# iucario/WorkoutDetector

Hardware: AMD Instinct MI355X
Metric: clips/sec (8x3x224x224 TSM-R50) (higher is better)
Workload: dtype f32

## Files before the change

workoutdetector_amd/csrc/tsm_conv_rules.h:

```cpp
#pragma once
#include <stdint.h>
#include <string.h>

#if defined(__HIPCC__)
#define TSM_HOST_DEVICE __host__ __device__
#else
#define TSM_HOST_DEVICE
#endif

namespace tsm {

struct ConvParams {
  const float *x;
  const float *w;
  const float *bias;
  const float *res;
  float *y;
  int N, Hi, Wi, C, logC4;
  int Ho, Wo, Cout;
  int stride, pad;
  int Kp;
  int M;
  int relu;
  int T;
  int fold;
  int ntm, ntn;
  int tile;
  int prec;
  const float *x2;
  int C2, Hi2, Wi2, stride2;
  int K1;
  int kseg_len;
  int ksplit;
  int tail_from;
  float *ypart;
  int reverse;
  int pos_major;
};

enum ConvPrec { kPrecF32 = 0, kPrecBf16x3 = 1, kPrecBf16 = 2 };
constexpr int kPrecBlockShift = 4;
constexpr int kPrecPosMajor = 8;

enum ConvTile {
  kTileAuto = 0, kTile128x128 = 1, kTile128x64 = 2, kTile64x64 = 3, kTile32x32 = 4,
  kTile128x128w8 = 5,
  kTile256x256 = 6,
  kTileWs = 7,
  kTile256x256p = 8,
  kNumTiles = 9
};

struct Fused23Params {
  const float *x;
  const float *w2;
  const float *bias2;
  const float *w3f;
  const float *bias3;
  const float *res;
  float *y;
  int N, H, W;
  int M;
  int kseg_len;
  int reverse;
};

struct BneckParams {
  const void *x;
  const void *w1;
  const float *bias1;
  const void *w2;
  const float *bias2;
  const void *w3;
  const float *bias3;
  void *y;
  int cin;
  int N, H, W;
  int T, fold;
  int reverse;
};

struct FrontParams {
  const void *x;
  const void *w1;
  const float *bias1;
  const void *w2;
  const float *bias2;
  void *y;
  int N, H, W;
  int T, fold;
  int reverse;
};

struct Conv31Params {
  const void *t2;
  const void *w3;
  const float *bias3;
  const void *res;
  void *y;
  const void *w1;
  const float *bias1;
  void *t1;
  int n_clips, T, HW;
  int K3, C, N1;
  int fold;
  int reverse;
  int log_px;
};

constexpr int kBK = 32;

inline void conv_tile_dims(int tile, int *bm, int *bn) {
  *bm = (tile == kTile256x256 || tile == kTile256x256p || tile == kTileWs) ? 256 : tile == kTile32x32 ? 32 : (tile == kTile64x64 ? 64 : 128);
  *bn = (tile == kTile256x256 || tile == kTile256x256p) ? 256 : tile == kTile32x32 ? 32 : ((tile == kTile128x128 || tile == kTile128x128w8) ? 128 : 64);
}

inline int conv_tile_from_name(const char *name) {
  if (!name) return kTileAuto;
  static const struct { const char *n; int t; } names[] = {{"128x128", kTile128x128}, {"128x64", kTile128x64},
      {"64x64", kTile64x64}, {"32x32", kTile32x32}, {"128x128w8", kTile128x128w8}, {"256x256", kTile256x256}, {"ws", kTileWs}, {"256x256p", kTile256x256p}};
  for (const auto &e : names)
    if (strcmp(name, e.n) == 0) return e.t;
  return kTileAuto;
}

inline int conv_num_segments(const ConvParams &p) {
  if (p.kseg_len <= 0) return 1;
  const int nk = p.Kp / kBK;
  return (int)(((long)nk + p.kseg_len - 1) / p.kseg_len);
}

inline void conv_tile_shape(const ConvParams &p, int *bm, int *bn) {
  const int bn128 = p.Cout % 128 == 0 ? 128 : 64;
  const bool few = (((long)p.M + 127) / 128) * (p.Cout / bn128) < 256;
  *bm = few ? 64 : 128;
  *bn = few ? 64 : bn128;
}

constexpr int kWsRounds = 11;
constexpr int kWsPatchMax = kWsRounds * 32;
constexpr int kW8Rounds = 6;
constexpr int kW8PatchMax = kW8Rounds * 32;
constexpr int kS2PatchMax = 289;

inline bool ws_tile_geometry(int H, int W, int *tr_out, int *tc_out, int max_px = 256, int max_patch = kWsPatchMax) {
  long best_tiles = -1;
  int best_tr = 0, best_tc = 0, best_patch = 0;
  for (int tc = 4; tc <= 128; ++tc) {
    int tr = max_px / tc;
    if (tr > H) tr = H;
    if (tr < 1) continue;
    const int patch = (tr + 2) * (tc + 2);
    if (patch > max_patch) continue;
// ... 165 lines not shown
inline bool conv1x1_ws_valid(const ConvParams &p) {
  return p.prec == kPrecBf16 && (p.C == 64 || p.C == 256) && p.Cout == 64 && p.Kp == p.C && p.stride == 1 && p.pad == 0 &&
         p.Hi == p.Ho && p.Wi == p.Wo && !p.res && !p.x2 && p.kseg_len == 0 && (double)p.M * 128.0 < 2.0e9 &&
         (p.T == 0 || (p.N % p.T == 0 && p.fold % 8 == 0 && 2 * (int64_t)p.fold <= p.C)) &&
         (double)(128 + 2.0 * p.Hi * p.Wi) * p.C * 2.0 < 2.0e9;
}
inline bool conv1x1_wsn_valid(const ConvParams &p, int n_cu) {
  if (p.prec != kPrecBf16 || p.stride != 1 || p.pad != 0 || p.Hi != p.Ho || p.Wi != p.Wo || p.res || p.kseg_len != 0) return false;
  if ((double)(128 + 2.0 * p.Hi * p.Wi) * p.C * 2.0 >= 2.0e9) return false;
  if (p.x2) {
    const bool l1 = p.C == 64 && p.C2 == 64 && p.K1 == 64 && p.Kp == 128 && p.Cout == 256;
    const bool l2 = p.C == 128 && p.C2 == 256 && p.K1 == 128 && p.Kp == 384 && p.Cout == 512 && n_cu >= 16;
    return p.T == 0 && (l1 || l2) && (double)(128.0 / ((double)p.Hi * p.Wi) + 2.0) * p.Hi2 * p.Wi2 * p.C2 * 2.0 < 2.0e9;
  }
  if (p.Kp != p.C) return false;
  if (p.T > 0 && (p.N % p.T != 0 || p.fold % 8 != 0 || 2 * (int64_t)p.fold > p.C)) return false;
  return (p.C == 256 && p.Cout == 128) || (p.C == 512 && p.Cout == 128) || (p.C == 512 && p.Cout == 256);
}

inline bool conv_tile_valid(const ConvParams &p, int tile, int n_cu) {
  if (p.T > 0 && (p.res || p.x2 || (p.pad == 0 && p.stride != 1)) &&
      (tile == kTile256x256 || tile == kTileWs || (tile == kTile256x256p && (p.pad != 0 || !(p.res || p.x2)))))
    return false;
  switch (tile) {
    case kTile128x128: return p.Cout % 128 == 0;
    case kTile128x64:
    case kTile64x64: return p.Cout % 64 == 0;
    case kTile32x32: return p.Cout % 32 == 0 && p.prec == kPrecF32;
    case kTile128x128w8: return p.Cout % 128 == 0;
    case kTile256x256:
    case kTile256x256p:
      return p.prec == kPrecBf16 && p.Cout % 256 == 0 && p.C % 64 == 0 && !(p.res && p.x2) && (p.pad != 1 || (!p.res && p.T == 0)) &&
             (!p.x2 || (p.K1 % 64 == 0 && p.C2 % 64 == 0)) && (tile == kTile256x256 || (p.Cout <= 2048 && p.Kp >= 128));
    case kTileWs: {
      int tr, tc;
      return conv3x3_ws_valid(p, &tr, &tc) || conv3x3_ws128s2_valid(p, &tr, &tc) || conv3x3_ws128_valid(p, &tr, &tc, nullptr) ||
             conv1x1_ws_valid(p) || conv1x1_wsn_valid(p, n_cu);
    }
    default: return false;
  }
}

enum ConvFamily { kFamInvalid = 0, kFamIgemm, kFamIgemmSeg, kFamBf16_256, kFamBf16_256p, kFamWs3x3, kFamWs128, kFamWs128s2, kFamWs1x1, kFamWsn };

struct ConvRoute {
  int family = kFamInvalid, ks = 0;
  int bm = 0, bn = 0, wgm = 0, wgn = 0;
  bool shift = false, res = false, dual = false, block_shift = false;
  bool pos_major = false;
  int ntm = 0, ntn = 0;
  long tiles = 0;
  unsigned grid = 0;
  int tr = 0, tc = 0, swz = 0;
};

inline bool conv_args_refused(const ConvParams &p, int ks) {
  const int kc = p.prec == kPrecBf16 ? 64 : kBK;
  if (p.Cout % 64 != 0 || p.Kp % kc != 0 || p.M <= 0) return true;
  if (p.logC4 < 0 || p.logC4 > 28 || (1 << p.logC4) * 4 != p.C) return true;
  if (ks != 7 && p.C % kc != 0) return true;
  if (p.T > 0 && ((ks != 1 && ks != 3) || (ks == 3 && p.kseg_len > 0) || p.N % p.T != 0 || p.fold % 4 != 0 ||
                  (p.res && 2 * (int64_t)p.fold > p.Cout) || (p.x2 && 2 * (int64_t)p.fold > p.C2)))
    return true;
  if (p.x2 && (ks != 1 || p.res || p.K1 % kc != 0 || p.C2 % kc != 0 || (int64_t)p.K1 + p.C2 != p.Kp || p.K1 != p.C))
    return true;
  if (p.x2 && (128.0 / ((double)p.Ho * p.Wo) + 4.0) * (double)p.Hi2 * p.Wi2 * p.C2 * 4.0 > 2.0e9) return true;
// ... 47 lines not shown
  else conv_tile_dims(p.tile, &r.bm, &r.bn);
  if (p.tile == kTile256x256 || p.tile == kTile256x256p) {
    const bool persistent = p.tile == kTile256x256p;
    if (!(persistent ? conv_bf16_256p_valid(p, ks) : conv_bf16_256_valid(p, ks))) return refused;
    r.family = persistent ? kFamBf16_256p : kFamBf16_256;
    r.wgm = 2; r.wgn = 4;
    r.shift = ks == 1 && p.T > 0;
    r.ntm = (int)(((long)p.M + 255) / 256); r.ntn = p.Cout / 256;
    r.tiles = (long)r.ntm * r.ntn;
    const int slots = n_cu & ~7;
    r.grid = (unsigned)(!persistent || r.tiles < slots || slots < 8 ? r.tiles : slots);
    return r.tiles > 0x7fffffffL ? refused : r;
  }
  if (p.tile == kTileWs) {
    if (ks == 3) {
      r.family = conv3x3_ws128s2_valid(p, &r.tr, &r.tc) ? kFamWs128s2 : conv3x3_ws128_valid(p, &r.tr, &r.tc, &r.swz) ? kFamWs128 :
                 conv3x3_ws_valid(p, &r.tr, &r.tc) ? kFamWs3x3 : kFamInvalid;
      if (r.family == kFamInvalid) return refused;
      if (r.family == kFamWs128s2) r.swz = ws128s2_swap(r.tr, r.tc);
      r.tiles = ws_frame_tiles(p.N, p.Ho, p.Wo, r.tr, r.tc);
    } else {
      r.family = ks != 1 || r.res ? kFamInvalid : conv1x1_ws_valid(p) ? kFamWs1x1 : conv1x1_wsn_valid(p, n_cu) ? kFamWsn : kFamInvalid;
      if (r.family == kFamInvalid) return refused;
      const int px = r.family == kFamWs1x1 || p.Kp <= 256 ? 128 : 64;
      r.tiles = ((long)p.M + px - 1) / px;
    }
    r.grid = persistent_grid(r.tiles, n_cu);
    if (r.family == kFamWsn && p.x2 && p.Kp == 384) {
      const int pairs = n_cu >> 4 << 3;
      r.grid = 2u * (unsigned)(r.tiles < pairs ? (r.tiles + 7) / 8 * 8 : pairs);
    }
    return r;
  }
  if (p.kseg_len > 0 && r.bm != 32) r.bm = r.bn = 64;
  if (r.bm == 32 && p.prec != kPrecF32) return refused;
  r.wgm = r.bm == 32 ? 1 : r.bm == 128 && r.bn == 128 && p.tile == kTile128x128w8 ? 4 : 2;
  r.wgn = r.bm == 32 ? 1 : 2;
  r.ntm = (int)(((long)p.M + r.bm - 1) / r.bm); r.ntn = p.Cout / r.bn;
  r.tiles = (long)r.ntm * r.ntn;
  long grid = r.tiles;
  if (p.kseg_len > 0) {
    if (r.res || ks == 7 || (r.shift && ks == 3)) return refused;
    if (p.ksplit == 2 && (p.tail_from <= 0 || p.tail_from >= r.tiles || p.tail_from % r.ntn != 0)) return refused;
    r.family = kFamIgemmSeg;
    r.pos_major = p.pos_major != 0 && r.bm == 64 && pos_major_valid(p, ks);
    grid = p.ksplit == 2 ? p.tail_from + (r.tiles - p.tail_from) * conv_num_segments(p) : r.tiles * (p.ksplit ? conv_num_segments(p) : 1);
  } else {
    r.family = kFamIgemm;
  }
  r.block_shift = p.T > 0 && (r.dual || r.res);
  r.grid = (unsigned)grid;
  return grid > 0x7fffffffL ? refused : r;
}

inline bool conv23_ws_valid(int n, int h, int w, int *tr_out = nullptr, int *tc_out = nullptr) {
  int tr, tc;
  return n > 0 && h > 0 && w > 0 && (double)h * w * 512.0 < 2.0e9 && (double)n * h * w < 2.0e9 &&
         ws_tile_geometry(h, w, tr_out ? tr_out : &tr, tc_out ? tc_out : &tc);
}
inline bool bneck_ws_valid(int cin, int n, int h, int w, int T, int fold) {
  return (cin == 256 || cin == 64) && n > 0 && h > 0 && w >= 1 && w <= 64 && (double)h * w * 512.0 * 3.0 < 2.0e9 &&
         (T == 0 || (T > 0 && n % T == 0 && fold == cin / 8));
}
inline bool front_s2_valid(int n, int h, int w, int T, int fold) {
  return n > 0 && h >= 2 && (h & 1) == 0 && w >= 2 && w <= 64 && (double)h * w * 512.0 * 3.0 < 2.0e9 &&
         (T == 0 || (T > 0 && n % T == 0 && fold == 32));
// ... 16 lines not shown
```

workoutdetector_amd/csrc/tsm_engine.hip:

```cpp
#include <hip/hip_runtime.h>

#include <sys/stat.h>

#include <algorithm>
#include <cerrno>
#include <cmath>
#include <cstdio>
#include <cstdlib>
#include <cstring>
#include <map>
#include <string>
#include <vector>

#include "../../include/tsm_hip.h"
#include "tsm_host_util.h"
#include "tsm_kernels.h"

#ifndef TSM_BUILD_ID
#define TSM_BUILD_ID __DATE__ "/" __TIME__
#endif

namespace {

using namespace tsm_host;
// ... 142 lines not shown
  hipStream_t stream = nullptr;
  bool finalized = false;
  int prec = tsm::kPrecF32;
  float *d_tap = nullptr;
  std::map<std::string, HostTensor> tensors;
  std::vector<ConvLayer> convs;
  std::vector<Block> blocks;
  float *d_fcw = nullptr, *d_fcb = nullptr;
  float *d_in = nullptr;
  float *d_in4 = nullptr;
  float *buf[5] = {nullptr, nullptr, nullptr, nullptr, nullptr};
  float *d_pooled = nullptr, *d_logits = nullptr;
  float *d_partial = nullptr;
  size_t partial_elems = 0;
  size_t buf_elems = 0;
  int h1 = 0, w1 = 0, hp = 0, wp = 0;
  hipEvent_t ev0 = nullptr, ev1 = nullptr;
  bool have_time = false;
  std::vector<void *> allocs;
  bool poison = false;
  std::vector<GuardBuf> guards;
  std::map<int, std::vector<int>> tile_cache;
  bool autotune = true;
  bool stem_pool = true;
  bool stem_direct = true;
  bool stem_planar = true;
  std::string tune_path, tune_sig;
  int force_tile = 0, force_code = -1;
  int fuse23 = -1;
  int fuse_block = -1;
  int fuse31 = -1;
  int fuse_front = -1;
  bool pos_major = true;
  int walk = -1;
  int n_cu = 256;
  int timing_left = 0;
  bool timing_only3x3 = false;
  std::vector<std::vector<hipEvent_t>> timing;
  std::vector<hipEvent_t> event_pool;
  std::vector<hipEvent_t> *cur_timing = nullptr;
};

namespace {

int fail(tsm_engine *e, int code, const std::string &msg) {
  if (e) e->err = msg; else g_create_error = msg;
  return code;
}

#define TSM_HIP(e, call)                                                                        \
  do {                                                                                          \
    hipError_t _st = (call);                                                                    \
    if (_st != hipSuccess)                                                                      \
      return fail((e), TSM_ERR_HIP, std::string(#call) + ": " + hipGetErrorString(_st));        \
  } while (0)

int add_conv(tsm_engine *e, const std::string &wkey, const std::string &bnp, int cin, int cout, int k, int stride, bool segmented) {
  ConvLayer c;
  static_cast<LayerGeom &>(c) = layer_geometry(cin, k, stride, e->prec);
  if (!segmented) c.kseg = 0;
  c.wkey = wkey; c.bnp = bnp; c.cin = cin; c.cout = cout; c.k = k; c.stride = stride;
  e->convs.push_back(c);
  return (int)e->convs.size() - 1;
}

void build_convnext_topology(tsm_engine *e) {
// ... 580 lines not shown

hipError_t Forward::launch_code(tsm::ConvParams p, int ks, int code) {
  return launch_conv_code(p, ks, code, e->d_partial, e->partial_elems, e->n_cu, s);
}

int Forward::conv(int idx, tsm::ConvParams p, int ks, bool is3x3) {
  p.reverse = next_dir();
  if (!tuning) {
    int code = tiles ? (*tiles)[idx] : 0;
    if (e->force_tile) code = e->force_tile;
    if (e->force_code >= 0) code = e->force_code;
    TSM_LAUNCH_K(e, s, is3x3, launch_code(p, ks, checked_code(p, code, e->n_cu)));
    return TSM_OK;
  }
  std::vector<int> cands;
  if (p.kseg_len > 0) {
    const size_t need = (size_t)tsm::conv_num_segments(p) * p.M * p.Cout;
    const long tiles64 = (long)((p.M + 63) / 64) * (p.Cout / 64);
    for (int t : {(int)tsm::kTile64x64, (int)tsm::kTile32x32}) {
      cands.push_back(t);
      if (need <= e->partial_elems && tiles64 < 4L * e->n_cu) cands.push_back(t | kCodeSplitK);
    }
    int tail_from = 0;
    const bool tail = tail_split_from(p, e->n_cu, e->partial_elems, &tail_from);
    if (tail) cands.push_back((int)tsm::kTile64x64 | kCodeTailK);
    tsm::ConvParams q = p;
    q.tile = tsm::kTile64x64;
    if (e->pos_major && tsm::pos_major_valid(q, ks)) {
      cands.push_back((int)tsm::kTile64x64 | kCodePosMajor);
      if (tail) cands.push_back((int)tsm::kTile64x64 | kCodePosMajor | kCodeTailK);
    }
  } else {
    for (int t = 1; t < tsm::kNumTiles; ++t)
      if (tsm::conv_tile_valid(p, t, e->n_cu)) cands.push_back(t);
  }
  float best_ms = 0.f;
  int best = 0;
  for (int t : cands) {
    float ms = 0.f;
    const int rc = time_best_of(e, s, [&] { return launch_code(p, ks, t); }, &ms);
    if (rc) return rc;
    if (best == 0 || ms < best_ms) {
      best = t;
      best_ms = ms;
    }
  }
  (*tiles)[idx] = best;
  return TSM_OK;
}

int Forward::run_basic(size_t k, int nn, float *x, float *y, int hh, int ww) {
  const Block &blk = e->blocks[k];
  const std::string &name = blk.name;
  const ConvLayer &c1 = e->convs[blk.conv1], &c2 = e->convs[blk.conv2];
  const int T = blk.T, shiftT = e->cfg.is_shift ? T : 0;
  const int ho = conv_out_size(hh, 3, blk.stride), wo = conv_out_size(ww, 3, blk.stride);
  const float *identity = x;
  if (blk.down >= 0) {
    tsm::ConvParams pd = make_params(e->convs[blk.down], x, nullptr, idb, nn, hh, ww, false, block_shift(e) ? shiftT : 0,
                                     e->cfg.shift_div, prec);
    int rcd = conv(blk.down, pd, 1, false);
    if (rcd) return rcd;
    identity = idb;
  }
  tsm::ConvParams p1 = make_params(c1, x, nullptr, t1, nn, hh, ww, true, shiftT, e->cfg.shift_div, prec);
  int rc1 = conv(blk.conv1, p1, 3, true);
  if (rc1) return rc1;
// ... 854 lines not shown
  if (!cfg || !out) return fail(nullptr, TSM_ERR_INVALID_ARG, "cfg/out is NULL");
  *out = nullptr;
  if (cfg->struct_size != (int32_t)sizeof(tsm_config))
    return fail(nullptr, TSM_ERR_INVALID_ARG, "tsm_config.struct_size mismatch (ABI)");
  if (cfg->num_class <= 0 || cfg->num_segments <= 0 || cfg->max_clips <= 0)
    return fail(nullptr, TSM_ERR_INVALID_ARG, "num_class, num_segments, max_clips must be positive");
  if (cfg->height < 32 || cfg->width < 32)
    return fail(nullptr, TSM_ERR_INVALID_ARG, "height/width must be >= 32");
  {
    const int64_t rows = (int64_t)cfg->max_clips * cfg->num_segments * ((cfg->height + 1) / 2) * ((cfg->width + 1) / 2);
    if (rows >= (int64_t)1 << 31)
      return fail(nullptr, TSM_ERR_CAPACITY, "max_clips * num_segments * (H/2) * (W/2) must stay below 2^31");
  }
  if (const char *why = shift_div_refusal(cfg->shift_div, tsm::kPrecF32)) return fail(nullptr, TSM_ERR_UNSUPPORTED, why);
  if (prec_of_dtype(cfg->dtype) < 0)
    return fail(nullptr, TSM_ERR_UNSUPPORTED, "dtype must be TSM_DTYPE_F32, TSM_DTYPE_BF16X3 or TSM_DTYPE_BF16");
  if (const char *why = shift_div_refusal(cfg->shift_div, prec_of_dtype(cfg->dtype))) return fail(nullptr, TSM_ERR_UNSUPPORTED, why);
  int ndev = 0;
  hipError_t st = hipGetDeviceCount(&ndev);
  if (st != hipSuccess || ndev <= 0)
    return fail(nullptr, TSM_ERR_HIP, std::string("no HIP device: ") + hipGetErrorString(st));
  if (cfg->device_id < 0 || cfg->device_id >= ndev) return fail(nullptr, TSM_ERR_INVALID_ARG, "bad device_id");
  tsm_engine *e = new tsm_engine();
  e->cfg = *cfg;
  e->prec = prec_of_dtype(cfg->dtype);
  const auto on = [](const char *s) { return atoi(s) != 0; };
  env_read("TSM_AUTOTUNE", &e->autotune, on);
  env_read("TSM_STEM_DIRECT", &e->stem_direct, on);
  env_read("TSM_STEM_POOL", &e->stem_pool, on);
  env_read("TSM_STEM_PLANAR", &e->stem_planar, on);
  env_read("TSM_CONV_TILE", &e->force_tile, tsm::conv_tile_from_name);
  env_read("TSM_CONV_CODE", &e->force_code, atoi);
  env_read("TSM_POS_MAJOR", &e->pos_major, on);
  env_read("TSM_FUSE_CONV23", &e->fuse23, on);
  env_read("TSM_FUSE_BLOCK", &e->fuse_block, on);
  env_read("TSM_FUSE_C3C1", &e->fuse31, on);
  env_read("TSM_FUSE_FRONT", &e->fuse_front, on);
  env_read("TSM_WALK", &e->walk, on);
  env_read("TSM_POISON", &e->poison, on);
  const char *tc = getenv("TSM_TUNE_CACHE");
  if (!tc) e->tune_path = default_tune_cache_path();
  else if (*tc && strcmp(tc, "0") != 0 && strcmp(tc, "off") != 0) e->tune_path = tc;
  build_topology(e);
  st = hipSetDevice(cfg->device_id);
  if (st == hipSuccess) st = hipStreamCreateWithFlags(&e->stream, hipStreamNonBlocking);
  if (st == hipSuccess) st = hipDeviceGetAttribute(&e->n_cu, hipDeviceAttributeMultiprocessorCount, cfg->device_id);
  if (st == hipSuccess) st = hipEventCreate(&e->ev0);
  if (st == hipSuccess) st = hipEventCreate(&e->ev1);
  if (st != hipSuccess) {
    g_create_error = std::string("engine init: ") + hipGetErrorString(st);
    delete e;
    return TSM_ERR_HIP;
  }
  if (!e->tune_path.empty()) {
    hipDeviceProp_t prop;
    e->tune_sig = "abi" + std::to_string(TSM_ABI_VERSION) + " build " TSM_BUILD_ID " " +
                  (hipGetDeviceProperties(&prop, cfg->device_id) == hipSuccess ? std::string(prop.gcnArchName) : "?") +
                  " cu" + std::to_string(e->n_cu) +
                  " T" + std::to_string(cfg->num_segments) + " " + std::to_string(cfg->height) + "x" +
                  std::to_string(cfg->width) + " dtype" + std::to_string(cfg->dtype) + " shift" +
                  std::to_string(cfg->is_shift ? cfg->shift_div : 0) + " fuse" + std::to_string(e->fuse23) + "/" + std::to_string(e->fuse_block) + "/" + std::to_string(e->fuse31) + "/" + std::to_string(e->fuse_front) +
                  " stem" + std::to_string(e->stem_direct ? 1 : 0) +
                  std::to_string(e->stem_pool ? 1 : 0) + std::to_string(e->stem_planar ? 1 : 0);
    e->tune_sig_base = e->tune_sig.size();
  }
  *out = e;
// ... 764 lines not shown
```

workoutdetector_amd/csrc/tsm_igemm.hip:

```cpp
#include "tsm_device.h"

namespace tsm {

template <int BM, int BN, int WGM, int WGN, int KS, bool SHIFT, bool RES, int PREC, bool DUAL = false, bool SEG = false>
__global__ void __launch_bounds__(64 * WGM * WGN, (SEG && BM == 64) ? ((PREC & kPrecBlockShift) ? 4 : 5) : 1)
conv_igemm(const ConvParams p) {
  constexpr bool BSHIFT = (PREC & kPrecBlockShift) != 0;
  constexpr bool POSM = (PREC & kPrecPosMajor) != 0;
  constexpr int PMODE = PREC & ~(kPrecBlockShift | kPrecPosMajor);
  static_assert(!POSM || (SEG && KS == 3 && BM == 64 && BN == 64 && !SHIFT && !RES && !DUAL && !BSHIFT && PMODE == kPrecF32),
                "position-major rows: the segmented fp32 3x3 on 64x64 tiles only (pos_major_valid)");
  static_assert(!BSHIFT || (!SHIFT && !RES), "block placement: a shifted identity (DUAL = false) or a shifted second source");
  constexpr bool RESID = RES || (BSHIFT && !DUAL);
  static_assert(!SEG || (PMODE == kPrecF32 && !RES && WGM * WGN <= 4 && BM == BN && BM <= 64),
                "segmented K accumulation: fp32, 64x64 / 32x32 tiles, no residual (ConvParams::kseg_len)");
  static_assert(WGM * WGN == 4 || WGM * WGN == 1 || WGM * WGN == 8,
                "4 waves per workgroup, 1 (32x32 small-M tiles) or 8 (128x128 with 4 waves per SIMD at 2 workgroups/CU)");
  constexpr int NT = 64 * WGM * WGN;
  constexpr int LRP = NT / 8;
  static_assert(!DUAL || (KS == 1 && !SHIFT && !RES), "K-concatenated second source: plain 1x1 convs only");
  constexpr bool X3 = PMODE == kPrecBf16x3;
  constexpr bool BF = PMODE == kPrecBf16;
  constexpr int EB = BF ? 2 : 4;
  constexpr int KC = 128 / EB;
  static_assert(!SHIFT || KS == 1 || (KS == 3 && !SEG), "the temporal shift is fused into 1x1 and unsegmented 3x3 convs only");
  constexpr int WTM = BM / WGM, WTN = BN / WGN;
  constexpr int TM = WTM / 32, TN = WTN / 32;
  constexpr int APASS = BM / LRP, BPASS = BN / LRP;
  constexpr bool RK = PMODE == kPrecF32 && ((BM == 64 && BN == 64) || (BM == 32 && BN == 32));
  constexpr int NBUF = RK ? 1 : 2;
  constexpr int CLD = BN + 4;
  static_assert(TM >= 1 && TN >= 1, "wave tile must hold at least one 32x32 MFMA tile");
  constexpr int SMEM_FLOATS = NBUF * (BM + BN) * kLds > BM * CLD ? NBUF * (BM + BN) * kLds : BM * CLD;

  __shared__ __attribute__((aligned(16))) float smem[SMEM_FLOATS];

  const int tid = threadIdx.x;
  const int lane = tid & 63;
  const int wave = tid >> 6;
  const int wm = wave / WGN, wn = wave % WGN;
  const int half = lane >> 5, l31 = lane & 31;

  const int bid = blockIdx.x;
  const bool tail_mode = SEG && p.ksplit == 2;
  const bool in_tail = tail_mode && bid >= p.tail_from;
  const int nwg = tail_mode ? p.tail_from : (int)gridDim.x;
  const int q = nwg >> 3, r = nwg & 7, xcd = bid & 7;
  int tile = (xcd < r ? xcd * (q + 1) : r * (q + 1) + (xcd - r) * q) + (bid >> 3);
  if (p.reverse) tile = nwg - 1 - tile;
  int seg = 0;
  if (SEG && p.ksplit == 1) {
    seg = tile / (p.ntm * p.ntn);
    tile -= seg * (p.ntm * p.ntn);
  }
  if (in_tail) {
    const int u = bid - p.tail_from, n_tail = p.ntm * p.ntn - p.tail_from;
    seg = u / n_tail;
    tile = p.tail_from + (u - seg * n_tail);
  }
  const bool split_wg = SEG && (p.ksplit == 1 || in_tail);
  const int tm = tile / p.ntn, tn = tile - tm * p.ntn;
  const int m0 = tm * BM, n0 = tn * BN;

  const int HoWo = p.Ho * p.Wo;
// ... 253 lines not shown
  u32x4 af16[4][TM], bf16f[4][TN];
  auto frag_load_bf = [&](int buf, int qg) {
    const float *As = smem + buf * (BM + BN) * kLds + (wm * WTM + l31) * kLds + qg * 8 + half * 4;
    const float *Bs = smem + buf * (BM + BN) * kLds + BM * kLds + (wn * WTN + l31) * kLds + qg * 8 + half * 4;
#pragma unroll
    for (int i = 0; i < TM; ++i) af16[qg][i] = *reinterpret_cast<const u32x4 *>(As + i * 32 * kLds);
#pragma unroll
    for (int j = 0; j < TN; ++j) bf16f[qg][j] = *reinterpret_cast<const u32x4 *>(Bs + j * 32 * kLds);
  };
  constexpr int NMFMA_BF = TM * TN;
  auto mfma_bf = [&](int qg, int item0, int nitems, auto &&inject) {
    int cnt = 0;
#pragma unroll
    for (int i = 0; i < TM; ++i)
#pragma unroll
      for (int j = 0; j < TN; ++j) {
        acc[i][j] = __builtin_amdgcn_mfma_f32_32x32x16_bf16(__builtin_bit_cast(bf16x8, af16[qg][i]),
                                                            __builtin_bit_cast(bf16x8, bf16f[qg][j]), acc[i][j], 0, 0, 0);
        ++cnt;
        const int done = (cnt * nitems) / NMFMA_BF, before = ((cnt - 1) * nitems) / NMFMA_BF;
#pragma unroll
        for (int it = before; it < done; ++it) {
          inject(item0 + it);
          __builtin_amdgcn_sched_barrier(0);
        }
      }
  };

  constexpr int EW = (X3 || BF) ? 8 : 4;
  constexpr int TPR = BN / EW;
  constexpr int RPP = NT / TPR;
  constexpr int EPASS = BM / RPP;
  const int ecol = (tid % TPR) * EW, erow = tid / TPR;
  f32x4 rres[(RESID && !X3 && !BF) ? EPASS : 1];
  u32x4 rres_h[(RESID && (X3 || BF)) ? EPASS : 1], rres_l[(RESID && X3) ? EPASS : 1];
  if (RESID && (X3 || BF) && !BSHIFT) {
    const size_t r_bytes = ((size_t)p.M - m0) * p.Cout * EB;
    const __amdgpu_buffer_rsrc_t rsrcR = buffer_window(reinterpret_cast<const char *>(p.res) + (size_t)m0 * p.Cout * EB, r_bytes);
#pragma unroll
    for (int k = 0; k < EPASS; ++k) {
      const unsigned o = (unsigned)(((erow + k * RPP) * p.Cout + n0 + ecol) * EB);
      rres_h[k] = __builtin_amdgcn_raw_buffer_load_b128(rsrcR, (int)o, 0, 0);
      if (X3) rres_l[k] = __builtin_amdgcn_raw_buffer_load_b128(rsrcR, (int)(o + 16), 0, 0);
    }
  }
  if (RESID && !X3 && !BF && !BSHIFT) {
    const size_t r_bytes = ((size_t)p.M - m0) * p.Cout * 4;
    const __amdgpu_buffer_rsrc_t rsrcR = buffer_window(p.res + (size_t)m0 * p.Cout, r_bytes);
#pragma unroll
    for (int k = 0; k < EPASS; ++k)
      rres[k] = buf_load4(rsrcR, (unsigned)(((erow + k * RPP) * p.Cout + n0 + ecol) * 4), 0);
  }
  if constexpr (RESID && BSHIFT) {
    const int rbase = m0 >= HoWo ? m0 - HoWo : 0;
    const int c = n0 + ecol;
    const int sel = c < p.fold ? 1 : c < 2 * p.fold ? -1 : 0;
    const unsigned step = (unsigned)(HoWo * p.Cout * EB);
    const size_t r_bytes = ((size_t)p.M - rbase) * p.Cout * EB;
    const __amdgpu_buffer_rsrc_t rsrcR = buffer_window(reinterpret_cast<const char *>(p.res) + (size_t)rbase * p.Cout * EB, r_bytes);
#pragma unroll
    for (int k = 0; k < EPASS; ++k) {
      const int rr = erow + k * RPP;
      const int t = ((m0 + rr) / HoWo) % p.T;
      unsigned o = (unsigned)(((m0 - rbase + rr) * p.Cout + c) * EB);
      if (sel > 0) o = t < p.T - 1 ? o + step : kInvalid;
      if (sel < 0) o = t > 0 ? o - step : kInvalid;
      if constexpr (X3 || BF) {
        rres_h[k] = __builtin_amdgcn_raw_buffer_load_b128(rsrcR, (int)o, 0, 0);
        if (X3) rres_l[k] = __builtin_amdgcn_raw_buffer_load_b128(rsrcR, (int)(o + 16), 0, 0);
      } else {
        rres[k] = buf_load4(rsrcR, o, 0);
      }
    }
  }

  int kt0 = 0, nk = p.Kp / KC;
  if (split_wg) {
    kt0 = seg * p.kseg_len;
    nk = kt0 + p.kseg_len < nk ? kt0 + p.kseg_len : nk;
// ... 28 lines not shown
#pragma unroll
    for (int it = 0; it < NITEMS; ++it) gload_item(k0, pm_first, it);
#pragma unroll
    for (int it = 0; it < NITEMS; ++it) lstore_item(0, it);
    const KStep k1 = kstep(pm_second, nk);
#pragma unroll
    for (int it = 0; it < NITEMS; ++it) gload_item(k1, pm_second, it);
  }
  __syncthreads();
  if constexpr (BF) {
    frag_load_bf(0, 0);
    frag_load_bf(0, 1);
    for (int kt = kt0; kt < nk; ++kt) {
      const int cur = (kt - kt0) & 1;
      const KStep k2 = kstep(kt + 2, nk);
      frag_load_bf(cur, 2);
      frag_load_bf(cur, 3);
      auto inject = [&](int it) {
        if (it < NITEMS) lstore_item(cur ^ 1, it);
        else gload_item(k2, kt + 2, it - NITEMS);
      };
      mfma_bf(0, 0, NITEMS, inject);
      mfma_bf(1, NITEMS, NITEMS, inject);
      __syncthreads();
      __builtin_amdgcn_sched_barrier(0);
      mfma_bf(2, 0, 0, [](int) {});
      frag_load_bf(cur ^ 1, 0);
      __builtin_amdgcn_sched_barrier(0);
      mfma_bf(3, 0, 0, [](int) {});
      __builtin_amdgcn_sched_barrier(0);
      frag_load_bf(cur ^ 1, 1);
      __builtin_amdgcn_sched_barrier(0);
    }
  } else if constexpr (RK) {
    f32x4 ra_[4], rb_[4];
    const bool trim = KS == 7 && p.Kp == 224 && nk == 7;
    const int nk_full = trim ? nk - 1 : nk;
    if constexpr (POSM) {
      int kt = pm_first, kt1 = pm_second;
      while (kt < nk) {
        const int bound = (kt / seg_len + 1) * seg_len, kend = bound < nk ? bound : nk;
        while (kt < kend) {
          const int kt2 = next_live_kstep(kt1 + 1, pm_live, pm_spt, nk);
          const KStep k2 = kstep(kt2, nk);
          {
            const float *As = smem + (wm * WTM + l31) * kLds + half * 4;
            const float *Bs = smem + BM * kLds + (wn * WTN + l31) * kLds + half * 4;
#pragma unroll
            for (int kk = 0; kk < 4; ++kk) {
              ra_[kk] = *reinterpret_cast<const f32x4 *>(As + kk * 8);
              rb_[kk] = *reinterpret_cast<const f32x4 *>(Bs + kk * 8);
            }
          }
          __syncthreads();
          int cnt = 0;
#pragma unroll
          for (int kk = 0; kk < 4; ++kk)
#pragma unroll
            for (int s4 = 0; s4 < 4; ++s4) {
              acc[0][0] = __builtin_amdgcn_mfma_f32_32x32x2f32(ra_[kk][s4], rb_[kk][s4], acc[0][0], 0, 0, 0);
              ++cnt;
              const int done = cnt < 12 ? (cnt * 2 * NITEMS) / 12 : 2 * NITEMS;
              const int before = cnt - 1 < 12 ? ((cnt - 1) * 2 * NITEMS) / 12 : 2 * NITEMS;
#pragma unroll
              for (int it = before; it < done; ++it) {
                if (it < NITEMS) lstore_item(0, it);
// ... 203 lines not shown
        if (r.block_shift) TSM_KLAUNCH_WALK(p.reverse, (conv_igemm<BM, BN, WGM, WGN, 1, false, false, kPrecF32 | kPrecBlockShift, true, true>), grid, block, 0, s, p);
        else TSM_KLAUNCH_WALK(p.reverse, (conv_igemm<BM, BN, WGM, WGN, 1, false, false, kPrecF32, true, true>), grid, block, 0, s, p);
        return hipGetLastError();
      }
    }
    if constexpr (BM == 64 && WGM == 2 && KS == 3 && !SHIFT) {
      if (r.pos_major) {
        TSM_KLAUNCH_WALK(p.reverse, (conv_igemm<64, 64, 2, 2, 3, false, false, kPrecF32 | kPrecPosMajor, false, true>), grid, block, 0, s, p);
        return hipGetLastError();
      }
    }
    TSM_KLAUNCH_WALK(p.reverse, (conv_igemm<BM, BN, WGM, WGN, KS, SHIFT, false, kPrecF32, false, true>), grid, block, 0, s, p);
    return hipGetLastError();
  }
}

template <int BM, int BN, int WGM, int WGN, int KS, bool SHIFT, bool RES>
static hipError_t launch_conv_t(const ConvParams &p, const ConvRoute &r, hipStream_t s) {
  if (r.family == kFamIgemmSeg) {
    if constexpr (!RES && KS != 7 && !(SHIFT && KS == 3)) return launch_conv_seg<BM, BN, WGM, WGN, KS, SHIFT>(p, r, s);
    else return hipErrorInvalidValue;
  }
  const dim3 grid(r.grid), block(64 * WGM * WGN);
  if constexpr (KS == 1 && !SHIFT && !RES) {
    if (r.dual && r.block_shift) TSM_LAUNCH_IGEMM_AND_RETURN(TSM_ARM_DUAL_SHIFT);
    if (r.dual) TSM_LAUNCH_IGEMM_AND_RETURN(TSM_ARM_DUAL);
  }
  if constexpr (RES && !SHIFT && KS != 7) {
    if (r.block_shift) TSM_LAUNCH_IGEMM_AND_RETURN(TSM_ARM_RES_SHIFT);
  }
  TSM_LAUNCH_IGEMM_AND_RETURN(TSM_ARM_PLAIN);
}

template <int KS, bool SHIFT, bool RES>
static hipError_t launch_conv_ks(const ConvParams &p, const ConvRoute &r, hipStream_t s) {
  if (r.bm == 32) return launch_conv_t<32, 32, 1, 1, KS, SHIFT, RES>(p, r, s);
  if (r.bm == 128 && r.bn == 128 && r.wgm == 4) return launch_conv_t<128, 128, 4, 2, KS, SHIFT, RES>(p, r, s);
  if (r.bm == 128 && r.bn == 128) return launch_conv_t<128, 128, 2, 2, KS, SHIFT, RES>(p, r, s);
  if (r.bm == 128) return launch_conv_t<128, 64, 2, 2, KS, SHIFT, RES>(p, r, s);
  return launch_conv_t<64, 64, 2, 2, KS, SHIFT, RES>(p, r, s);
}

hipError_t launch_conv(const ConvParams &p_in, int ks, hipStream_t s) {
  const bool device = p_in.tile == kTile256x256 || p_in.tile == kTile256x256p || p_in.tile == kTileWs;
  const DeviceInfo *di = device ? &device_info() : nullptr;
  const ConvRoute r = conv_route(p_in, ks, di ? di->n_cu : 0);
  if (r.family == kFamInvalid) return hipErrorInvalidValue;
  if (di && di->status != hipSuccess) return di->status;
  ConvParams p = p_in;
  p.ntm = r.ntm; p.ntn = r.ntn;
  if (r.family == kFamBf16_256 || r.family == kFamBf16_256p) return launch_conv_bf16_256(p, r, s);
  if (r.family >= kFamWs3x3) return launch_conv_ws(p, r, s);
  if (p.ksplit == 2 && !p.ypart) return hipErrorInvalidValue;
  if (ks == 1) return r.res ? launch_conv_ks<1, false, true>(p, r, s) : r.shift ? launch_conv_ks<1, true, false>(p, r, s) : launch_conv_ks<1, false, false>(p, r, s);
  if (ks == 3) return r.res ? launch_conv_ks<3, false, true>(p, r, s) : r.shift ? launch_conv_ks<3, true, false>(p, r, s) : launch_conv_ks<3, false, false>(p, r, s);
  return launch_conv_ks<7, false, false>(p, r, s);
}

__global__ void __launch_bounds__(256) splitk_reduce_kernel(const float *__restrict__ partial, int n_seg, int64_t n4,
                                                            int64_t seg_stride4, int cout4,
                                                            const float *__restrict__ bias, const float *__restrict__ res,
                                                            float *__restrict__ y, int relu) {
  const int64_t stride = (int64_t)gridDim.x * blockDim.x;
  const float floor_ = relu ? 0.f : -INFINITY;
  const f32x4 *p4 = reinterpret_cast<const f32x4 *>(partial);
  for (int64_t i = (int64_t)blockIdx.x * blockDim.x + threadIdx.x; i < n4; i += stride) {
    f32x4 t = p4[i];
    for (int sgm = 1; sgm < n_seg; ++sgm) t += p4[i + sgm * seg_stride4];
    f32x4 v = t + reinterpret_cast<const f32x4 *>(bias)[i % cout4];
    if (res) v += reinterpret_cast<const f32x4 *>(res)[i];
    v[0] = fmaxf(v[0], floor_);
    v[1] = fmaxf(v[1], floor_);
    v[2] = fmaxf(v[2], floor_);
    v[3] = fmaxf(v[3], floor_);
    reinterpret_cast<f32x4 *>(y)[i] = v;
  }
}


__global__ void __launch_bounds__(256) splitk_reduce_pos_kernel(const float *__restrict__ partial, int n_seg, int64_t n4,
                                                                int64_t seg_stride4, int cout4, int m_first, int n_frames,
                                                                int howo, const float *__restrict__ bias,
                                                                float *__restrict__ y, int relu) {
  const int64_t stride = (int64_t)gridDim.x * blockDim.x;
  const float floor_ = relu ? 0.f : -INFINITY;
  const f32x4 *p4 = reinterpret_cast<const f32x4 *>(partial);
// ... 37 lines not shown
```

workoutdetector_amd/engine.py:

```python
from __future__ import annotations

import ctypes as C
from dataclasses import dataclass
from typing import Dict, List, Mapping, Optional, Sequence

import numpy as np

from . import _lib
from .weights import (BACKBONES, CONVNEXT, CONVNEXT_DEPTHS, CONVNEXT_WIDTHS, DEPTHS, NL_BLOCKS, SHIFT_PLACES, TDN, TDN_FRAMES, WIDTHS,
                      _convnext_depths, _tdn_depths, feature_width, is_convnext, is_mmaction_state_dict, make_state_dict, make_tdn_state_dict,
                      remap_checkpoint_keys, remap_mmaction_keys, remap_tdn_keys, remap_timm_keys, remap_torchvision_keys, tdn_alpha_beta)

CONSENSUS_TYPES = {'avg': 0, 'identity': 1}


@dataclass
class NodeArg:
    name: str
    shape: list
    type: str = 'tensor(float)'


def _as_f32(a) -> np.ndarray:
    return np.ascontiguousarray(np.asarray(a), dtype=np.float32)
# ... 419 lines not shown
                    names += ['fuse2'] if (li, b) == (2, 0) else []
                    names += ([p + '.downsample'] if b == 0 else []) + [p + '.conv1']
                    names += [p + part for part in ('.mse_squeeze', '.mse_diff', '.mse_s2', '.mse_mix', '.mse_excite_shift')] if li >= 2 else []
                    names += [p + '.conv2', p + '.conv3']
            return names + ['head']
        if self.convnext_depths:
            names = ['pack_input', 'stem.pack', 'stem.conv', 'stem.norm']
            for s, nb in enumerate(self.convnext_depths):
                names += [f'stages.{s}.downsample.norm', f'stages.{s}.downsample'] if s else []
                for b in range(nb):
                    names += [f'stages.{s}.blocks.{b}' + part for part in ('.dwln', '.fc1', '.gelu', '.fc2')]
            return names + ['head.pool', 'head.norm', 'head']
        names = ['pack_input', 'conv1', 'maxpool']
        blocks, kind = BACKBONES[self.base_model]
        for li, nb in enumerate(blocks, start=1):
            for b in range(nb):
                p = f'layer{li}.{b}'
                if kind == 'basic':
                    names += ([p + '.downsample'] if b == 0 and li > 1 else []) + [p + '.conv1', p + '.conv2']
                else:
                    names += ([p + '.downsample'] if b == 0 else []) + [p + '.conv1', p + '.conv2', p + '.conv3']
                    if self.non_local and (li, b) in NL_BLOCKS:
                        names += [p + '.nl.qkv', p + '.nl.pool', p + '.nl.attn', p + '.nl.W']
            if self.temporal_pool and li == 1:
                names.append('layer2.tpool')
        return names + ['head']

    @property
    def tdn_chunk_clips(self) -> int:
        per_clip = (self.height // 4) * (self.width // 4) * self.num_segments * 1024
        return max(1, min(8, self.max_clips, ((1 << 29) - 1) // per_clip))

    TILE_NAMES = {0: 'heuristic', 1: '128x128', 2: '128x64', 3: '64x64', 4: '32x32', 5: '128x128w8', 6: '256x256', 7: 'ws',
                  8: '256x256p'}

    @classmethod
    def tile_name(cls, code: int) -> str:
        return (cls.TILE_NAMES[code & 15] + ('/pos' if code & 0x80 else '') + ('/splitK' if code & 0x100 else '') + ('/tailK' if code & 0x200 else '') + ('+conv3' if code & 0x400 else '') +
                ('+block' if code & 0x800 else '') + ('+conv1' if code & 0x1000 else '') + ('+conv2' if code & 0x2000 else ''))

    def conv_tiles(self, n_clips: int) -> Dict[str, str]:
        buf = (C.c_int32 * 256)()
        n = C.c_int32()
        _lib.check(self._lib.tsm_conv_tiles(self._h, n_clips, buf, 256, C.byref(n)), self._h)
        if self.tdn_depths:
            names = ['conv1', 'diff.conv1_5'] + [k for k in self.launch_names() if k.startswith(('resnext_layer1.', 'layer'))
                                                 and k.endswith(('.downsample', '.conv1', '.conv2', '.conv3'))]
            assert n.value == len(names)
            return {k: self.tile_name(buf[i]) for i, k in enumerate(names)}
        if self.convnext_depths:
            names = [k for k in self.launch_names() if k == 'stem.conv' or k.endswith(('.downsample', '.fc1', '.fc2'))]
            assert n.value == len(names)
            return {k: self.tile_name(buf[i]) for i, k in enumerate(names)}
        names = [k for k in self.launch_names() if k not in ('pack_input', 'maxpool', 'head', 'layer2.tpool') and not k.endswith(('.nl.pool', '.nl.attn'))]
        assert n.value == len(names)
        return {k: self.tile_name(buf[i]) for i, k in enumerate(names)}

    def set_layer_timing(self, n_forwards: int, only_conv3x3: bool = False) -> None:
        _lib.check(self._lib.tsm_set_layer_timing(self._h, n_forwards, int(only_conv3x3)), self._h)

    def layer_times_ms(self, forward_index: int) -> Dict[str, float]:
        buf = (C.c_float * 512)()
        n = C.c_int32()
        _lib.check(self._lib.tsm_layer_times(self._h, forward_index, C.addressof(buf), 512, C.byref(n)), self._h)
        names = self.launch_names()
        assert n.value == len(names), (n.value, len(names))
        return {k: float(buf[i]) for i, k in enumerate(names)}
# ... 692 lines not shown
```

Before: 1912.

## Add 64x128 fp32 igemm tile for 1x1 convs with single-buffered LDS pipeline

Adds a new 64x128 tile variant for unsegmented fp32 1x1 convolutions. It has its own single-buffered main loop that interleaves LDS stores and global loads between MFMA steps, and a two-half epilogue that stages results through LDS while prefetching the residual. The tile joins the autotune candidate set, toggled by an environment flag, with a higher occupancy launch bound. It gives the autotuner a mid-size shape for layers where 128x128 launches too few blocks and 64x64 gives too little reuse. The cost is more kernel instantiations and longer tuning.

```diff
diff --git a/workoutdetector_amd/csrc/tsm_conv_rules.h b/workoutdetector_amd/csrc/tsm_conv_rules.h
--- a/workoutdetector_amd/csrc/tsm_conv_rules.h
+++ b/workoutdetector_amd/csrc/tsm_conv_rules.h
@@ -48,7 +48,8 @@
   kTile256x256 = 6,
   kTileWs = 7,
   kTile256x256p = 8,
-  kNumTiles = 9
+  kTile64x128 = 9,
+  kNumTiles = 10
 };
 
 struct Fused23Params {
@@ -111,14 +112,14 @@
 constexpr int kBK = 32;
 
 inline void conv_tile_dims(int tile, int *bm, int *bn) {
-  *bm = (tile == kTile256x256 || tile == kTile256x256p || tile == kTileWs) ? 256 : tile == kTile32x32 ? 32 : (tile == kTile64x64 ? 64 : 128);
-  *bn = (tile == kTile256x256 || tile == kTile256x256p) ? 256 : tile == kTile32x32 ? 32 : ((tile == kTile128x128 || tile == kTile128x128w8) ? 128 : 64);
+  *bm = (tile == kTile256x256 || tile == kTile256x256p || tile == kTileWs) ? 256 : tile == kTile32x32 ? 32 : ((tile == kTile64x64 || tile == kTile64x128) ? 64 : 128);
+  *bn = (tile == kTile256x256 || tile == kTile256x256p) ? 256 : tile == kTile32x32 ? 32 : ((tile == kTile128x128 || tile == kTile128x128w8 || tile == kTile64x128) ? 128 : 64);
 }
 
 inline int conv_tile_from_name(const char *name) {
   if (!name) return kTileAuto;
   static const struct { const char *n; int t; } names[] = {{"128x128", kTile128x128}, {"128x64", kTile128x64},
-      {"64x64", kTile64x64}, {"32x32", kTile32x32}, {"128x128w8", kTile128x128w8}, {"256x256", kTile256x256}, {"ws", kTileWs}, {"256x256p", kTile256x256p}};
+      {"64x64", kTile64x64}, {"32x32", kTile32x32}, {"128x128w8", kTile128x128w8}, {"256x256", kTile256x256}, {"ws", kTileWs}, {"256x256p", kTile256x256p}, {"64x128", kTile64x128}};
   for (const auto &e : names)
     if (strcmp(name, e.n) == 0) return e.t;
   return kTileAuto;
@@ -350,6 +351,9 @@
     case kTile256x256p:
       return p.prec == kPrecBf16 && p.Cout % 256 == 0 && p.C % 64 == 0 && !(p.res && p.x2) && (p.pad != 1 || (!p.res && p.T == 0)) &&
              (!p.x2 || (p.K1 % 64 == 0 && p.C2 % 64 == 0)) && (tile == kTile256x256 || (p.Cout <= 2048 && p.Kp >= 128));
+    case kTile64x128:
+      return p.prec == kPrecF32 && p.pad == 0 && p.kseg_len == 0 && p.Cout % 128 == 0 &&
+             !(p.T > 0 && (p.res || p.x2 || p.stride != 1));
     case kTileWs: {
       int tr, tc;
       return conv3x3_ws_valid(p, &tr, &tc) || conv3x3_ws128s2_valid(p, &tr, &tc) || conv3x3_ws128_valid(p, &tr, &tc, nullptr) ||
@@ -463,6 +467,7 @@
     }
     return r;
   }
+  if (p.tile == kTile64x128 && ks != 1) return refused;
   if (p.kseg_len > 0 && r.bm != 32) r.bm = r.bn = 64;
   if (r.bm == 32 && p.prec != kPrecF32) return refused;
   r.wgm = r.bm == 32 ? 1 : r.bm == 128 && r.bn == 128 && p.tile == kTile128x128w8 ? 4 : 2;
diff --git a/workoutdetector_amd/csrc/tsm_engine.hip b/workoutdetector_amd/csrc/tsm_engine.hip
--- a/workoutdetector_amd/csrc/tsm_engine.hip
+++ b/workoutdetector_amd/csrc/tsm_engine.hip
@@ -198,6 +198,7 @@
   int fuse31 = -1;
   int fuse_front = -1;
   bool pos_major = true;
+  bool tile_64x128 = true;
   int walk = -1;
   int n_cu = 256;
   int timing_left = 0;
@@ -844,7 +845,7 @@
     }
   } else {
     for (int t = 1; t < tsm::kNumTiles; ++t)
-      if (tsm::conv_tile_valid(p, t, e->n_cu)) cands.push_back(t);
+      if (tsm::conv_tile_valid(p, t, e->n_cu) && (t != tsm::kTile64x128 || e->tile_64x128)) cands.push_back(t);
   }
   float best_ms = 0.f;
   int best = 0;
@@ -1765,6 +1766,7 @@
   env_read("TSM_CONV_TILE", &e->force_tile, tsm::conv_tile_from_name);
   env_read("TSM_CONV_CODE", &e->force_code, atoi);
   env_read("TSM_POS_MAJOR", &e->pos_major, on);
+  env_read("TSM_TILE_64X128", &e->tile_64x128, on);
   env_read("TSM_FUSE_CONV23", &e->fuse23, on);
   env_read("TSM_FUSE_BLOCK", &e->fuse_block, on);
   env_read("TSM_FUSE_C3C1", &e->fuse31, on);
diff --git a/workoutdetector_amd/csrc/tsm_igemm.hip b/workoutdetector_amd/csrc/tsm_igemm.hip
--- a/workoutdetector_amd/csrc/tsm_igemm.hip
+++ b/workoutdetector_amd/csrc/tsm_igemm.hip
@@ -3,7 +3,7 @@
 namespace tsm {
 
 template <int BM, int BN, int WGM, int WGN, int KS, bool SHIFT, bool RES, int PREC, bool DUAL = false, bool SEG = false>
-__global__ void __launch_bounds__(64 * WGM * WGN, (SEG && BM == 64) ? ((PREC & kPrecBlockShift) ? 4 : 5) : 1)
+__global__ void __launch_bounds__(64 * WGM * WGN, (SEG && BM == 64) ? ((PREC & kPrecBlockShift) ? 4 : 5) : (BM == 64 && BN == 128) ? 4 : 1)
 conv_igemm(const ConvParams p) {
   constexpr bool BSHIFT = (PREC & kPrecBlockShift) != 0;
   constexpr bool POSM = (PREC & kPrecPosMajor) != 0;
@@ -28,8 +28,11 @@
   constexpr int TM = WTM / 32, TN = WTN / 32;
   constexpr int APASS = BM / LRP, BPASS = BN / LRP;
   constexpr bool RK = PMODE == kPrecF32 && ((BM == 64 && BN == 64) || (BM == 32 && BN == 32));
-  constexpr int NBUF = RK ? 1 : 2;
-  constexpr int CLD = BN + 4;
+  constexpr bool RK2 = PMODE == kPrecF32 && BM == 64 && BN == 128;
+  static_assert(!RK2 || (WGM == 2 && WGN == 2 && KS == 1 && !SEG && !BSHIFT && !POSM),
+                "64x128 tiles: unsegmented fp32 1x1 convs on 2x2 waves, no block placement (conv_tile_valid)");
+  constexpr int NBUF = (RK || RK2) ? 1 : 2;
+  constexpr int CLD = RK2 ? 68 : BN + 4;
   static_assert(TM >= 1 && TN >= 1, "wave tile must hold at least one 32x32 MFMA tile");
   constexpr int SMEM_FLOATS = NBUF * (BM + BN) * kLds > BM * CLD ? NBUF * (BM + BN) * kLds : BM * CLD;
 
@@ -349,7 +352,7 @@
   constexpr int RPP = NT / TPR;
   constexpr int EPASS = BM / RPP;
   const int ecol = (tid % TPR) * EW, erow = tid / TPR;
-  f32x4 rres[(RESID && !X3 && !BF) ? EPASS : 1];
+  f32x4 rres[(RESID && !X3 && !BF && !RK2) ? EPASS : 1];
   u32x4 rres_h[(RESID && (X3 || BF)) ? EPASS : 1], rres_l[(RESID && X3) ? EPASS : 1];
   if (RESID && (X3 || BF) && !BSHIFT) {
     const size_t r_bytes = ((size_t)p.M - m0) * p.Cout * EB;
@@ -361,7 +364,7 @@
       if (X3) rres_l[k] = __builtin_amdgcn_raw_buffer_load_b128(rsrcR, (int)(o + 16), 0, 0);
     }
   }
-  if (RESID && !X3 && !BF && !BSHIFT) {
+  if (RESID && !X3 && !BF && !BSHIFT && !RK2) {
     const size_t r_bytes = ((size_t)p.M - m0) * p.Cout * 4;
     const __amdgpu_buffer_rsrc_t rsrcR = buffer_window(p.res + (size_t)m0 * p.Cout, r_bytes);
 #pragma unroll
@@ -456,6 +459,89 @@
       frag_load_bf(cur ^ 1, 1);
       __builtin_amdgcn_sched_barrier(0);
     }
+  } else if constexpr (RK2) {
+    f32x4 fa[4], fb[2][4];
+    auto frags = [&]() {
+      const float *As = smem + (wm * WTM + l31) * kLds + half * 4;
+      const float *Bs = smem + BM * kLds + (wn * WTN + l31) * kLds + half * 4;
+#pragma unroll
+      for (int kk = 0; kk < 4; ++kk) {
+        fa[kk] = *reinterpret_cast<const f32x4 *>(As + kk * 8);
+#pragma unroll
+        for (int j = 0; j < 2; ++j) fb[j][kk] = *reinterpret_cast<const f32x4 *>(Bs + j * 32 * kLds + kk * 8);
+      }
+    };
+    auto mfma_step = [&](auto &&inject) {
+      int cnt = 0;
+#pragma unroll
+      for (int kk = 0; kk < 4; ++kk)
+#pragma unroll
+        for (int s4 = 0; s4 < 4; ++s4)
+#pragma unroll
+          for (int j = 0; j < 2; ++j) {
+            acc[0][j] = __builtin_amdgcn_mfma_f32_32x32x2f32(fa[kk][s4], fb[j][kk][s4], acc[0][j], 0, 0, 0);
+            ++cnt;
+            const int done = cnt < 24 ? (cnt * 2 * NITEMS) / 24 : 2 * NITEMS;
+            const int before = cnt - 1 < 24 ? ((cnt - 1) * 2 * NITEMS) / 24 : 2 * NITEMS;
+#pragma unroll
+            for (int it = before; it < done; ++it) {
+              inject(it);
+              __builtin_amdgcn_sched_barrier(0);
+            }
+          }
+    };
+    for (int kt = kt0; kt < nk - 1; ++kt) {
+      const KStep k2 = kstep(kt + 2, nk);
+      frags();
+      __syncthreads();
+      mfma_step([&](int it) {
+        if (it < NITEMS) lstore_item(0, it);
+        else gload_item(k2, kt + 2, it - NITEMS);
+      });
+      __syncthreads();
+    }
+    frags();
+    __syncthreads();
+    const int hrow = tid >> 4, hcol = (tid & 15) * 4;
+    const int ocol = n0 + (hcol >> 5) * 64 + (hcol & 31);
+    f32x4 rr2[RES ? 2 : 1][RES ? 4 : 1];
+    auto res_half = [&](int h) {
+      if constexpr (RES) {
+        const size_t r_bytes = ((size_t)p.M - m0) * p.Cout * 4;
+        const __amdgpu_buffer_rsrc_t rsrcR = buffer_window(p.res + (size_t)m0 * p.Cout, r_bytes);
+#pragma unroll
+        for (int k = 0; k < 4; ++k) rr2[h][k] = buf_load4(rsrcR, (unsigned)(((hrow + 16 * k) * p.Cout + ocol + 32 * h) * 4), 0);
+      }
+    };
+    res_half(0);
+    mfma_step([](int) {});
+    __builtin_amdgcn_sched_barrier(0);
+    res_half(1);
+    const size_t y_bytes = ((size_t)p.M - m0) * p.Cout * 4;
+    const __amdgpu_buffer_rsrc_t rsrcY = buffer_window(reinterpret_cast<char *>(p.y) + (size_t)m0 * p.Cout * 4, y_bytes);
+    const float floor_ = p.relu ? 0.f : -INFINITY;
+#pragma unroll
+    for (int h = 0; h < 2; ++h) {
+      if (h) __syncthreads();
+#pragma unroll
+      for (int e = 0; e < 16; ++e)
+        smem[(wm * WTM + (e & 3) + 8 * (e >> 2) + 4 * half) * CLD + wn * 32 + l31] = acc[0][h][e];
+      __syncthreads();
+      const f32x4 bias = *reinterpret_cast<const f32x4 *>(p.bias + ocol + 32 * h);
+#pragma unroll
+      for (int k = 0; k < 4; ++k) {
+        const int rr = hrow + 16 * k;
+        f32x4 v = *reinterpret_cast<const f32x4 *>(smem + rr * CLD + hcol);
+        v += bias;
+        if constexpr (RES) v += rr2[h][k];
+        v[0] = fmaxf(v[0], floor_);
+        v[1] = fmaxf(v[1], floor_);
+        v[2] = fmaxf(v[2], floor_);
+        v[3] = fmaxf(v[3], floor_);
+        __builtin_amdgcn_raw_buffer_store_b128(__builtin_bit_cast(u32x4, v), rsrcY, (int)((rr * p.Cout + ocol + 32 * h) * 4), 0, 0);
+      }
+    }
+    return;
   } else if constexpr (RK) {
     f32x4 ra_[4], rb_[4];
     const bool trim = KS == 7 && p.Kp == 224 && nk == 7;
@@ -725,6 +811,16 @@
   TSM_LAUNCH_IGEMM_AND_RETURN(TSM_ARM_PLAIN);
 }
 
+static hipError_t launch_conv_64x128(const ConvParams &p, const ConvRoute &r, hipStream_t s) {
+  if (r.ks != 1 || r.family != kFamIgemm || r.block_shift || p.prec != kPrecF32) return hipErrorInvalidValue;
+  const dim3 grid(r.grid), block(256);
+  if (r.dual) TSM_KLAUNCH_WALK(p.reverse, (conv_igemm<64, 128, 2, 2, 1, false, false, kPrecF32, true>), grid, block, 0, s, p);
+  else if (r.res) TSM_KLAUNCH_WALK(p.reverse, (conv_igemm<64, 128, 2, 2, 1, false, true, kPrecF32>), grid, block, 0, s, p);
+  else if (r.shift) TSM_KLAUNCH_WALK(p.reverse, (conv_igemm<64, 128, 2, 2, 1, true, false, kPrecF32>), grid, block, 0, s, p);
+  else TSM_KLAUNCH_WALK(p.reverse, (conv_igemm<64, 128, 2, 2, 1, false, false, kPrecF32>), grid, block, 0, s, p);
+  return hipGetLastError();
+}
+
 template <int KS, bool SHIFT, bool RES>
 static hipError_t launch_conv_ks(const ConvParams &p, const ConvRoute &r, hipStream_t s) {
   if (r.bm == 32) return launch_conv_t<32, 32, 1, 1, KS, SHIFT, RES>(p, r, s);
@@ -745,6 +841,7 @@
   if (r.family == kFamBf16_256 || r.family == kFamBf16_256p) return launch_conv_bf16_256(p, r, s);
   if (r.family >= kFamWs3x3) return launch_conv_ws(p, r, s);
   if (p.ksplit == 2 && !p.ypart) return hipErrorInvalidValue;
+  if (r.bm == 64 && r.bn == 128) return launch_conv_64x128(p, r, s);
   if (ks == 1) return r.res ? launch_conv_ks<1, false, true>(p, r, s) : r.shift ? launch_conv_ks<1, true, false>(p, r, s) : launch_conv_ks<1, false, false>(p, r, s);
   if (ks == 3) return r.res ? launch_conv_ks<3, false, true>(p, r, s) : r.shift ? launch_conv_ks<3, true, false>(p, r, s) : launch_conv_ks<3, false, false>(p, r, s);
   return launch_conv_ks<7, false, false>(p, r, s);
diff --git a/workoutdetector_amd/engine.py b/workoutdetector_amd/engine.py
--- a/workoutdetector_amd/engine.py
+++ b/workoutdetector_amd/engine.py
@@ -475,7 +475,7 @@
         return max(1, min(8, self.max_clips, ((1 << 29) - 1) // per_clip))
 
     TILE_NAMES = {0: 'heuristic', 1: '128x128', 2: '128x64', 3: '64x64', 4: '32x32', 5: '128x128w8', 6: '256x256', 7: 'ws',
-                  8: '256x256p'}
+                  8: '256x256p', 9: '64x128'}
 
     @classmethod
     def tile_name(cls, code: int) -> str:
```

New measurement: 1939, median of 6. 1.01x the previous value.
